# zhuzhui-2000/mobilesuperresolution

Hardware: AMD Instinct MI355X
Metric: HR megapixels/sec (WDSR-B x4, 48x48 LR patches), full training step (higher is better)
Workload: dtype bf16; 1 GPU; WDSR-B x4, 16 blocks / 24 units, 48x48 LR patches, batch 32 per GPU, fwd+L1+bwd+Adam; global_batch=32, parallelism=dp1

## Files before the change

### include/sr_hotpath.h

```cpp
#ifndef SR_HOTPATH_H
#define SR_HOTPATH_H
#include <stddef.h>
#include <stdint.h>

#ifdef __cplusplus
extern "C" {
#endif

typedef void* sr_stream_t;

#define SR_DTYPE_F32 0
#define SR_DTYPE_BF16 1

int sr_abi_version(void);

int sr_wdsr_block_fwd(const void* x, void* y, const void* wblob, const float* cinit,
                      int N, int H, int W, int F, int dtype, sr_stream_t stream);

int sr_wdsr_block2_fwd(const void* x, void* ya, void* yb, const void* wblob_a, const void* wblob_b,
                       const float* cinit_a, const float* cinit_b, void* tsave_a, void* tsave_b, int N, int H, int W,
                       int F, int dtype, sr_stream_t stream);

int sr_wdsr_block2_bwd_data(const void* xa, const void* xb, const void* dyb, void* dxb, void* dxa,
                            const void* wblob_a, const void* wblob_b, const float* cinit_a, const float* cinit_b,
// ... 111 lines not shown

typedef struct { const int* idx; void* out; long src_off, src_stride; int n, reps, as_float; } sr_pack_seg_t;
typedef struct { const float* partial; const int* sidx; const int* dst; long dst_off, dst_stride, slab; int wgs, n, reps; } sr_unpack_seg_t;
int sr_param_pack(const float* flat, float* src, const int* chan_tab, int n_chan, const int* bias_tab, const float* bias_const,
                  int n_bias, const sr_pack_seg_t* segs, int nseg, int dtype, sr_stream_t stream);
int sr_param_grads(const float* flat, float* dsrc, float* gflat, const int* chan_tab, int n_chan, const int* bias_tab,
                   int n_bias, const sr_unpack_seg_t* segs, int nseg, sr_stream_t stream);

typedef struct {
  int F, NB, R, dtype, N, H, W;
  float mean;
  const float* flat; float* gflat;
  const int* chan_tab; int n_chan;
  const int* bias_tab; const float* bias_const; int n_bias;
  float* src; float* dsrc;
  long src_head_off, src_body_off, src_body_stride, src_tail_off;
  const int* idx_head; int n_idx_head;
  const int* idx_body; int n_idx_body;
  const int* idx_cinit; int n_idx_cinit;
  const int* idx_tail; int n_idx_tail;
  void* blob_head; void* blob_body; float* cinit_body; void* blob_tail;
  float* part_a; float* part_b; float* part_tail; float* part_head;
  int wgs_body, wgs_tail, wgs_head;
  int slab_a, slab_b, slab_tail, slab_head;
  const int* ga_sidx; const int* ga_dst; int n_ga;
  const int* gb_sidx; const int* gb_dst; int n_gb;
  const int* gt_sidx; const int* gt_dst; int n_gt;
  const int* gh_sidx; const int* gh_dst; int n_gh;
  const float* x; void* acts; void* grads; float* out; const float* dout;
  void* tsave; void* dtsave;
  const float* hr; int loss_kind; float loss_gscale; float* loss_part;
  int nb_split, chan_split, bias_split;
  int adam_in_wn_bwd;
} sr_wdsr_net_t;

#define SR_NET_SAVE_ACTS 1
#define SR_NET_WEIGHTS_PACKED 2
#define SR_NET_PACK_ONLY 4
int sr_wdsr_net_forward(const sr_wdsr_net_t* net, int flags, sr_stream_t stream);
int sr_wdsr_net_backward(const sr_wdsr_net_t* net, sr_stream_t stream);
int sr_wdsr_net_backward_part(const sr_wdsr_net_t* net, int part, sr_stream_t stream);

int sr_pixel_shuffle(const float* in, float* out, int N, int C, int H, int W, int r, int inverse, sr_stream_t stream);

int sr_tail_bwd_loss(const float* sr, const float* hr, int loss_kind, float gscale, float* loss_part, const void* feat,
                     const float* x_nchw, float mean, const void* wblob, void* dfeat, float* partial, int wgs, int N, int H,
                     int W, int F, int R, int dtype, sr_stream_t stream);

typedef struct { float w_lerp, beta2, one_minus_beta2, bc2_sqrt, eps, neg_step_size; } sr_adam_t;
int sr_adam_step(float* param, const float* grad, float* exp_avg, float* exp_avg_sq, long n, const sr_adam_t* a,
                 const float* loss_part, int n_loss, float loss_scale, float* loss_out, sr_stream_t stream);
int sr_loss_value(const float* loss_part, int n_loss, float loss_scale, float* loss_out, sr_stream_t stream);
int sr_scale_by(void* y, const void* x, long n, const float* scale, int dtype, sr_stream_t stream);
int sr_wdsr_net_train_step(const sr_wdsr_net_t* net, float* exp_avg, float* exp_avg_sq, long n_params, const sr_adam_t* a,
                           float loss_scale, float* loss_out, sr_stream_t stream);

int sr_conv7_fwd(const void* x, const void* wpacked, const float* bias, void* y, int N, int H, int W, int CIN, int COUT, int relu,
                 int out_f32, sr_stream_t stream);

int sr_probe_mfma_bf16(const void* a_frag, const void* b_frag, float* acc_out, sr_stream_t stream);
int sr_probe_mfma_f32(const float* a_frag, const float* b_frag, float* acc_out, sr_stream_t stream);
int sr_probe_tr_read(const void* img_bf16, int n_elems, const int* lane_elem_off, void* out_bf16x4,
                     sr_stream_t stream);
int sr_probe_copy(const void* src, void* dst, size_t n_bytes, sr_stream_t stream);
int sr_probe_launch_floor(void* out, int gx, int gy, int threads, int lds_bytes, int reps, sr_stream_t stream);
int sr_probe_launch_floor_graph(void* out, int gx, int gy, int threads, int lds_bytes, int reps, int iters,
// ... 8 lines not shown
```

### mobilesuperresolution_amd/_lib.py

```python
from __future__ import annotations

import ctypes
import os
from ctypes import c_int, c_size_t, c_void_p

import torch

_HERE = os.path.dirname(os.path.abspath(__file__))
LIB_PATH = os.environ.get("SR_HOTPATH_LIB_PATH") or os.path.join(
    _HERE, "libsr_hotpath_dbg.so" if os.environ.get("SR_HOTPATH_DEBUG_LIB") == "1" else "libsr_hotpath.so")
ABI_VERSION = 13
DTYPE_CODE = {torch.float32: 0, torch.bfloat16: 1}

_P, _I, _Z, _L, _F = c_void_p, c_int, c_size_t, ctypes.c_long, ctypes.c_float
SIGNATURES = {
    "sr_abi_version": ([], _I),
    "sr_wdsr_block_fwd": ([_P, _P, _P, _P, _I, _I, _I, _I, _I, _P], _I),
    "sr_wdsr_block2_fwd": ([_P] * 9 + [_I] * 5 + [_P], _I),
    "sr_wdsr_fwd_rs": ([_P] * 9 + [_I] * 6 + [_P], _I),
    "sr_conv7_fwd": ([_P] * 4 + [_I] * 7 + [_P], _I),
    "sr_wdsr_fwd_rs_repeat": ([_P] * 9 + [_I] * 7 + [_P], _I),
    "sr_wdsr_block_wgrad_saved": ([_P] * 8 + [_I] * 7 + [_L] * 5 + [_P], _I),
    "sr_wdsr_block2_bwd_data": ([_P] * 11 + [_I] * 5 + [_P], _I),
    "sr_wdsr_block2_fwd_repeat": ([_P] * 7 + [_I] * 6 + [_P], _I),
    "sr_probe_launch_floor": ([_P, _I, _I, _I, _I, _I, _P], _I),
    "sr_probe_launch_floor_graph": ([_P, _I, _I, _I, _I, _I, _I, _P, _P], _I),
    "sr_debug_set_stamps": ([_P, _L], _I),
    "sr_c3_trunk_fwd": ([_P] * 6 + [_I] * 7 + [_L, _P], _I),
    "sr_c3_trunk_bwd": ([_P] * 11 + [_I] * 8 + [_L, _P], _I),
    "sr_tail_bwd": ([_P, _P, _P, _F, _P, _P, _P] + [_I] * 7 + [_P], _I),
    "sr_nas_dw_wgrad": ([_P, _P, _P, _P, _I, _I, _I, _I, _I, _I, _P], _I),
    "sr_wdsr_block_fwd_repeat": ([_P, _P, _P, _P, _I, _I, _I, _I, _I, _I, _P], _I),
    "sr_wdsr_block_bwd_data": ([_P, _P, _P, _P, _P, _I, _I, _I, _I, _I, _P], _I),
    "sr_wdsr_block_wgrad": ([_P, _P, _P, _P, _P, _P, _I, _I, _I, _I, _I, _I, _I, _L, _L, _L, _L, _P], _I),
    "sr_wdsr_block_slab_sizes": ([_I, _P, _P], _I),
    "sr_head_fwd": ([_P, _P, _P, _F, _I, _I, _I, _I, _I, _P], _I),
    "sr_tail_fwd": ([_P, _P, _P, _P, _F, _I, _I, _I, _I, _I, _I, _P], _I),
    "sr_tail_bwd_data": ([_P, _P, _P, _I, _I, _I, _I, _I, _I, _P], _I),
    "sr_tail_wgrad": ([_P, _P, _P, _F, _P, _I, _I, _I, _I, _I, _I, _I, _P], _I),
    "sr_head_wgrad": ([_P, _P, _F, _P, _I, _I, _I, _I, _I, _I, _P], _I),
    "sr_c3_fwd": ([_P, _P, _P, _P, _I, _I, _I, _I, _I, _I, _P], _I),
    "sr_c3_bwd_data": ([_P, _P, _P, _P, _P, _I, _I, _I, _I, _I, _I, _P], _I),
    "sr_c3_wgrad": ([_P, _P, _P, _P, _I, _I, _I, _I, _I, _I, _I, _P], _I),
    "sr_flow_warp_fwd": ([_P, _P, _P, _I, _I, _I, _I, _P], _I),
# ... 10 lines not shown
    "sr_nas_body_fwd": ([_P, _P, _P, _L, _P, _L, _P, _L, _P, _L] + [_I] * 6 + [_P], _I),
    "sr_nas_body_bwd": ([_P] * 7 + [_L, _P, _L, _P, _L, _P, _L, _P, _L, _P, _L] + [_I] * 7 + [_P, _P], _I),
    "sr_psnr": ([_P, _P, _P, _P] + [_I] * 7 + [_P], _I),
    "sr_pixel_shuffle": ([_P, _P, _I, _I, _I, _I, _I, _I, _P], _I),
    "sr_tail_bwd_loss": ([_P, _P, _I, _F, _P, _P, _P, _F, _P, _P, _P] + [_I] * 7 + [_P], _I),
    "sr_adam_step": ([_P, _P, _P, _P, _L, _P, _P, _I, _F, _P, _P], _I),
    "sr_loss_value": ([_P, _I, _F, _P, _P], _I),
    "sr_scale_by": ([_P, _P, _L, _P, _I, _P], _I),
    "sr_wdsr_net_train_step": ([_P, _P, _P, _L, _P, _F, _P, _P], _I),
    "sr_wdsr_net_forward": ([_P, _I, _P], _I),
    "sr_wdsr_net_backward": ([_P, _P], _I),
    "sr_wdsr_net_backward_part": ([_P, _I, _P], _I),
    "sr_probe_mfma_bf16": ([_P, _P, _P, _P], _I),
    "sr_probe_mfma_f32": ([_P, _P, _P, _P], _I),
    "sr_probe_tr_read": ([_P, _I, _P, _P, _P], _I),
    "sr_probe_copy": ([_P, _P, _Z, _P], _I),
}

class WdsrNet(ctypes.Structure):
    _fields_ = (
        [(n, _I) for n in ("F", "NB", "R", "dtype", "N", "H", "W")] + [("mean", _F)] +
        [("flat", _P), ("gflat", _P), ("chan_tab", _P), ("n_chan", _I),
         ("bias_tab", _P), ("bias_const", _P), ("n_bias", _I), ("src", _P), ("dsrc", _P)] +
        [(n, _L) for n in ("src_head_off", "src_body_off", "src_body_stride", "src_tail_off")] +
        [("idx_head", _P), ("n_idx_head", _I), ("idx_body", _P), ("n_idx_body", _I),
         ("idx_cinit", _P), ("n_idx_cinit", _I), ("idx_tail", _P), ("n_idx_tail", _I),
         ("blob_head", _P), ("blob_body", _P), ("cinit_body", _P), ("blob_tail", _P),
         ("part_a", _P), ("part_b", _P), ("part_tail", _P), ("part_head", _P)] +
        [(n, _I) for n in ("wgs_body", "wgs_tail", "wgs_head", "slab_a", "slab_b", "slab_tail", "slab_head")] +
        [("ga_sidx", _P), ("ga_dst", _P), ("n_ga", _I), ("gb_sidx", _P), ("gb_dst", _P), ("n_gb", _I),
         ("gt_sidx", _P), ("gt_dst", _P), ("n_gt", _I), ("gh_sidx", _P), ("gh_dst", _P), ("n_gh", _I),
         ("x", _P), ("acts", _P), ("grads", _P), ("out", _P), ("dout", _P), ("tsave", _P), ("dtsave", _P),
         ("hr", _P), ("loss_kind", _I), ("loss_gscale", _F), ("loss_part", _P),
         ("nb_split", _I), ("chan_split", _I), ("bias_split", _I), ("adam_in_wn_bwd", _I)])


class C3Warp(ctypes.Structure):
    _fields_ = [("frame", _P), ("frame_bs", _L), ("state", _P), ("flow", _P), ("flow_bs", _L), ("flow_bound", _P),
                ("dstate", _P), ("dflow", _P), ("dflow_bs", _L), ("x0_save", _P)]


class C3Unpack(ctypes.Structure):
    _fields_ = [("sidx0", _P), ("dst0", _P), ("n0", _I), ("sidx1", _P), ("dst1", _P), ("n1", _I), ("gflat", _P)]


class PackSeg(ctypes.Structure):
    _fields_ = [("idx", _P), ("out", _P), ("src_off", _L), ("src_stride", _L), ("n", _I), ("reps", _I), ("as_float", _I)]


class UnpackSeg(ctypes.Structure):
    _fields_ = [("partial", _P), ("sidx", _P), ("dst", _P), ("dst_off", _L), ("dst_stride", _L), ("slab", _L), ("wgs", _I),
                ("n", _I), ("reps", _I)]


class AdamScalars(ctypes.Structure):
    _fields_ = [(n, _F) for n in ("w_lerp", "beta2", "one_minus_beta2", "bc2_sqrt", "eps", "neg_step_size")]


_lib = None


class HotpathError(RuntimeError):
    pass


def _declare(lib):
    for name, (args, res) in SIGNATURES.items():
# ... 92 lines not shown
```

### mobilesuperresolution_amd/csrc/sr_abi.hip

```cpp
#include <algorithm>
#include <cstdlib>
#include "../../include/sr_hotpath.h"
#include "wdsr_block.h"
#include "wdsr_fwd_rs.h"
#include "wdsr_fwd_stream.h"
#include "wdsr_bwd_rs.h"
#include "wdsr_bwd_pair_lds.h"
#include "wdsr_wgrad_rs.h"
#include "wdsr_ends.h"
#include "wdsr_prep.h"
#include "conv3x3.h"
#include "spynet_conv.h"
#include "nas_block.h"
#include "nas_dw_lc.h"
#include "nas_bwd_fused.h"
#include "flow_warp.h"
#include "metrics.h"
#include "patches.h"
#include "train_step.h"
#include "pixel_shuffle.h"

extern "C" int sr_abi_version(void) { return 13; }

#ifdef SR_DEBUG_STAMPS
#define SR_AB(name) (getenv(name) != nullptr)
#else
#define SR_AB(name) false
#endif

namespace {

template <typename T, int F, int E, int L>
int launch_block_fwd(const void* x, void* y, const void* wblob, const float* cinit, int N, int H, int W,
                     hipStream_t st, void* tsave = nullptr) {
  typedef BlockCfg<F, E, L> C;
  const int tiles_x = (W + C::TW - 1) / C::TW, tiles_y = (H + C::TH - 1) / C::TH;
  dim3 grid(tiles_x * tiles_y, N), block(64 * C::NPT_H);
  hipLaunchKernelGGL((wdsr_block_fwd_kernel<T, F, E, L>), grid, block, 0, st, (const T*)x, (T*)y, (const T*)wblob,
                     cinit, H, W, tiles_x, (T*)tsave);
  SR_HIP_CHECK_LAUNCH();
  return 0;
}

template <typename T, int F, int E, int L>
int launch_block_bwd_data(const void* x, const void* dy, void* dx, const void* wblob, const float* cinit, int N,
                          int H, int W, hipStream_t st, void* dtsave = nullptr) {
  typedef BlockCfg<F, E, L> C;
  const int tiles_x = (W + C::TW - 1) / C::TW, tiles_y = (H + C::TH - 1) / C::TH;
  dim3 grid(tiles_x * tiles_y, N), block(64 * C::NPT_O);
  hipLaunchKernelGGL((wdsr_block_bwd_data_kernel<T, F, E, L>), grid, block, 0, st, (const T*)x, (const T*)dy, (T*)dx,
                     (const T*)wblob, cinit, H, W, tiles_x, (T*)dtsave);
  SR_HIP_CHECK_LAUNCH();
  return 0;
}

// ... 812 lines not shown
                                   n->cinit_body + (size_t)(i + 1) * n->n_idx_cinit, ts ? ts + (size_t)i * side : nullptr,
                                   ts ? ts + (size_t)(i + 1) * side : nullptr, n->N, n->H, n->W, n->F, n->dtype, stream)))
        return rc;
      cur = nxt;
      ++i;
      continue;
    }
    char* nxt = save_acts ? acts + (size_t)(i + 1) * act : (cur == acts ? acts + act : acts);
    if (pairs) {
      char* ts = (save_acts && saved) ? (char*)n->tsave + (size_t)i * side : nullptr;
      if ((rc = sr_wdsr_fwd_rs(cur, nullptr, nxt, (char*)n->blob_body + i * blob, nullptr, n->cinit_body + (size_t)i * n->n_idx_cinit,
                               nullptr, ts, nullptr, 1, n->N, n->H, n->W, n->F, n->dtype, stream)))
        return rc;
      cur = nxt;
      continue;
    }
    if (save_acts && saved) {
      rc = n->F == 24 ? launch_block_fwd<__bf16, 24, 144, 20>(cur, nxt, (char*)n->blob_body + i * blob,
                                                              n->cinit_body + (size_t)i * n->n_idx_cinit, n->N, n->H, n->W,
                                                              st, (char*)n->tsave + (size_t)i * side)
                      : launch_block_fwd<__bf16, 32, 192, 26>(cur, nxt, (char*)n->blob_body + i * blob,
                                                              n->cinit_body + (size_t)i * n->n_idx_cinit, n->N, n->H, n->W,
                                                              st, (char*)n->tsave + (size_t)i * side);
      if (rc) return rc;
    } else if ((rc = sr_wdsr_block_fwd(cur, nxt, (char*)n->blob_body + i * blob,
                                       n->cinit_body + (size_t)i * n->n_idx_cinit, n->N, n->H, n->W, n->F, n->dtype, stream)))
      return rc;
    cur = nxt;
  }
  return sr_tail_fwd(cur, n->x, n->out, n->blob_tail, n->mean, n->N, n->H, n->W, n->F, n->R, n->dtype, stream);
}

namespace {
struct FusedAdam { float* m; float* v; AdamArgs a; const float* loss_part; int n_loss; float loss_scale; float* loss_out; };
}
static int net_backward_part_impl(const sr_wdsr_net_t* n, int part, sr_stream_t stream, const FusedAdam* fa) {
  if (!n || !n->flat || !n->gflat || !n->dsrc || !n->x || !n->acts || !n->grads || part < 0 || part > 2) return -2;
  if (part != 2 && (n->hr ? (!n->out || !n->loss_part || (n->loss_kind != 1 && n->loss_kind != 2)) : !n->dout)) return -2;
  hipStream_t st = (hipStream_t)stream;
  const size_t esz = n->dtype == SR_DTYPE_BF16 ? 2 : 4;
  const size_t act = (size_t)n->N * n->H * n->W * n->F * esz;
  const size_t blob = (size_t)n->n_idx_body * esz;
  const long act_e = (long)n->N * n->H * n->W * n->F;
  char* acts = (char*)n->acts;
  char* grads = (char*)n->grads;
  const bool pairs = net_uses_pairs(n) ||
                     (n->F == 32 && n->dtype == SR_DTYPE_BF16 && net_tiles(n) <= 384 && !getenv("SR_F32_ONE_BLOCK"));
  const bool saved = net_saves_side_images(n, true);
  const size_t side = side_image_bytes(n);
  int split = part == 0 ? 0 : n->nb_split;
  if (part != 0 && (split <= 0 || split >= n->NB || (pairs && ((n->NB - split) & 1)))) return -2;
  const int b0 = part == 1 ? split : 0, b1 = part == 2 ? split : n->NB;
  int rc;
  if (part != 2) {
    if (n->hr) {
      if ((rc = sr_tail_bwd_loss(n->out, n->hr, n->loss_kind, n->loss_gscale, n->loss_part, acts + (size_t)n->NB * act, n->x,
                                 n->mean, n->blob_tail, grads + (size_t)n->NB * act, n->part_tail, n->wgs_tail, n->N, n->H, n->W,
                                 n->F, n->R, n->dtype, stream)))
        return rc;
    } else if (n->dtype == SR_DTYPE_BF16) {
      if ((rc = sr_tail_bwd(n->dout, acts + (size_t)n->NB * act, n->x, n->mean, n->blob_tail, grads + (size_t)n->NB * act,
                            n->part_tail, n->wgs_tail, n->N, n->H, n->W, n->F, n->R, n->dtype, stream)))
        return rc;
    } else {
      if ((rc = sr_tail_bwd_data(n->dout, grads + (size_t)n->NB * act, n->blob_tail, n->N, n->H, n->W, n->F, n->R,
                                 n->dtype, stream)))
        return rc;
// ... 48 lines not shown
        return rc;
    } else if ((rc = sr_wdsr_block_wgrad(a0, g1, wb0, ci0, pa0, pb0, nl, wgs_part, n->N, n->H, n->W, n->F, n->dtype, act_e,
                                         act_e, (long)n->n_idx_body, (long)n->n_idx_cinit, stream)))
      return rc;
  }
  if (part != 1)
    if ((rc = sr_head_wgrad(grads, n->x, n->mean, n->part_head, n->wgs_head, n->N, n->H, n->W, n->F, n->dtype, stream)))
      return rc;
  {
    UnpackSegs us;
    us.nseg = 0;
    int blk = 0;
    auto add = [&](const float* part_, const int* sidx, const int* dst, long off, long stride, long slab, int wgs, int cnt,
                   int reps) {
      us.s[us.nseg++] = UnpackSeg{part_, sidx, dst, off, stride, slab, wgs, cnt, reps, blk};
      blk += reps * unpack_blocks(cnt, wgs);
    };
    if (nl > 0) {
      add(n->part_a, n->ga_sidx, n->ga_dst, n->src_body_off + b0 * n->src_body_stride, n->src_body_stride, n->slab_a, wgs_part,
          n->n_ga, nl);
      add(n->part_b, n->gb_sidx, n->gb_dst, n->src_body_off + b0 * n->src_body_stride, n->src_body_stride, n->slab_b, wgs_part,
          n->n_gb, nl);
    }
    if (part != 2) add(n->part_tail, n->gt_sidx, n->gt_dst, n->src_tail_off, 0, n->slab_tail, n->wgs_tail, n->n_gt, 1);
    if (part != 1) add(n->part_head, n->gh_sidx, n->gh_dst, n->src_head_off, 0, n->slab_head, n->wgs_head, n->n_gh, 1);
    hipLaunchKernelGGL(unpack_all_kernel, dim3(blk), dim3(64 * UNPACK_Q), 0, st, n->dsrc, us);
  }
  const int c0 = part == 1 ? n->chan_split : 0, c1 = part == 2 ? n->chan_split : n->n_chan;
  const int d0 = part == 1 ? n->bias_split : 0, d1 = part == 2 ? n->bias_split : n->n_bias;
  const int cb = (c1 - c0 + 3) / 4, bb = (d1 - d0 + 255) / 256;
  if (fa)
    hipLaunchKernelGGL(wn_bwd_adam_kernel, dim3(cb + bb), dim3(256), 0, st, const_cast<float*>(n->flat), n->dsrc, n->gflat, fa->m, fa->v,
                       (const int4*)n->chan_tab + c0, c1 - c0, n->bias_tab + 3 * d0, d1 - d0, cb, fa->a, fa->loss_part, fa->n_loss,
                       fa->loss_scale, fa->loss_out);
  else
    hipLaunchKernelGGL(wn_bwd_kernel, dim3(cb + bb), dim3(256), 0, st, n->flat, n->dsrc, n->gflat, (const int4*)n->chan_tab + c0,
                       c1 - c0, n->bias_tab + 3 * d0, d1 - d0, cb);
  SR_HIP_CHECK_LAUNCH();
  return 0;
}
extern "C" int sr_wdsr_net_backward_part(const sr_wdsr_net_t* n, int part, sr_stream_t stream) {
  return net_backward_part_impl(n, part, stream, nullptr);
}

extern "C" int sr_wdsr_net_backward(const sr_wdsr_net_t* n, sr_stream_t stream) { return sr_wdsr_net_backward_part(n, 0, stream); }

extern "C" int sr_param_pack(const float* flat, float* src, const int* chan_tab, int n_chan, const int* bias_tab,
                             const float* bias_const, int n_bias, const sr_pack_seg_t* segs, int nseg, int dtype,
                             sr_stream_t stream) {
  if (!flat || !src || !chan_tab || n_chan <= 0 || n_bias < 0 || (n_bias > 0 && (!bias_tab || !bias_const)) || !segs || nseg < 1 ||
      nseg > 4 || (dtype != SR_DTYPE_F32 && dtype != SR_DTYPE_BF16))
    return -2;
  hipStream_t st = (hipStream_t)stream;
  const int cb = (n_chan + 3) / 4, bb = (n_bias + 255) / 256;
  hipLaunchKernelGGL(wn_src_kernel, dim3(cb + bb), dim3(256), 0, st, flat, src, (const int4*)chan_tab, n_chan, bias_tab, bias_const,
                     n_bias, cb);
  PackSegs ps;
  ps.nseg = nseg;
  int blk = 0;
  for (int k = 0; k < nseg; ++k) {
    const sr_pack_seg_t& g = segs[k];
    if (!g.idx || !g.out || g.n <= 0 || g.reps <= 0) return -2;
    ps.s[k] = PackSeg{g.idx, g.out, g.src_off, g.src_stride, g.n, g.reps, g.as_float, blk};
    blk += g.reps * ((g.n + 255) / 256);
  }
  if (dtype == SR_DTYPE_BF16) hipLaunchKernelGGL((pack_all_kernel<__bf16>), dim3(blk), dim3(256), 0, st, src, ps);
  else hipLaunchKernelGGL((pack_all_kernel<float>), dim3(blk), dim3(256), 0, st, src, ps);
// ... 169 lines not shown
}

extern "C" int sr_adam_step(float* p, const float* g, float* m, float* v, long n, const sr_adam_t* a, const float* loss_part,
                            int n_loss, float loss_scale, float* loss_out, sr_stream_t stream) {
  if (!p || !g || !m || !v || !a || n <= 0 || (loss_out && (!loss_part || n_loss <= 0))) return -2;
  const AdamArgs aa{a->w_lerp, a->beta2, a->one_minus_beta2, a->bc2_sqrt, a->eps, a->neg_step_size};
  const long blocks = (n + 1023) / 1024;
  hipLaunchKernelGGL(adam_step_kernel, dim3((unsigned)blocks), dim3(256), 0, (hipStream_t)stream, p, g, m, v, n, aa, loss_part, n_loss,
                     loss_scale, loss_out);
  SR_HIP_CHECK_LAUNCH();
  return 0;
}
extern "C" int sr_loss_value(const float* loss_part, int n_loss, float loss_scale, float* loss_out, sr_stream_t stream) {
  if (!loss_part || !loss_out || n_loss <= 0) return -2;
  hipLaunchKernelGGL(loss_sum_kernel, dim3(1), dim3(64), 0, (hipStream_t)stream, loss_part, n_loss, loss_scale, loss_out);
  SR_HIP_CHECK_LAUNCH();
  return 0;
}
extern "C" int sr_scale_by(void* y, const void* x, long n, const float* scale, int dtype, sr_stream_t stream) {
  if (!y || !x || !scale || n <= 0 || ((uintptr_t)y & 15) || ((uintptr_t)x & 15)) return -2;
  const unsigned blocks = (unsigned)((n + 2047) / 2048);
  if (dtype == SR_DTYPE_BF16)
    hipLaunchKernelGGL(scale_by_kernel<__bf16>, dim3(blocks), dim3(256), 0, (hipStream_t)stream, (__bf16*)y, (const __bf16*)x, n, scale);
  else if (dtype == SR_DTYPE_F32)
    hipLaunchKernelGGL(scale_by_kernel<float>, dim3(blocks), dim3(256), 0, (hipStream_t)stream, (float*)y, (const float*)x, n, scale);
  else return -1;
  SR_HIP_CHECK_LAUNCH();
  return 0;
}
extern "C" int sr_wdsr_net_train_step(const sr_wdsr_net_t* n, float* m, float* v, long n_params, const sr_adam_t* a,
                                      float loss_scale, float* loss_out, sr_stream_t stream) {
  if (!n || !n->hr || !m || !v || !a || n_params <= 0) return -2;
  int rc;
  if ((rc = sr_wdsr_net_forward(n, SR_NET_SAVE_ACTS, stream))) return rc;
  static const bool separate = SR_AB("SR_TRAIN_SEPARATE_ADAM");
  if (!separate && n->adam_in_wn_bwd) {
    const FusedAdam fa{m, v, AdamArgs{a->w_lerp, a->beta2, a->one_minus_beta2, a->bc2_sqrt, a->eps, a->neg_step_size}, n->loss_part,
                       n->wgs_tail, loss_scale, loss_out};
    return net_backward_part_impl(n, 0, stream, &fa);
  }
  if ((rc = sr_wdsr_net_backward(n, stream))) return rc;
  return sr_adam_step(const_cast<float*>(n->flat), n->gflat, m, v, n_params, a, n->loss_part, n->wgs_tail, loss_scale, loss_out, stream);
}

__global__ void probe_mfma_bf16_kernel(const bf16x8* a, const bf16x8* b, float* out) {
  const int l = threadIdx.x;
  f32x16 acc = zero16();
  acc = mma16<__bf16>(a[l], b[l], acc);
#pragma unroll
  for (int i = 0; i < 16; ++i) out[l * 16 + i] = acc[i];
}
__global__ void probe_mfma_f32_kernel(const f32x8* a, const f32x8* b, float* out) {
  const int l = threadIdx.x;
  f32x16 acc = zero16();
  acc = mma16<float>(a[l], b[l], acc);
#pragma unroll
  for (int i = 0; i < 16; ++i) out[l * 16 + i] = acc[i];
}
__global__ void probe_tr_kernel(const __bf16* img, int n, const int* off, bf16x4* out) {
  __shared__ __attribute__((aligned(16))) __bf16 lds[8192];
  for (int i = threadIdx.x; i < n && i < 8192; i += 64) lds[i] = img[i];
  __syncthreads();
  typedef __attribute__((address_space(3))) bf16x4 lds_bf16x4;
  out[threadIdx.x] = __builtin_amdgcn_ds_read_tr16_b64_v4bf16((lds_bf16x4*)(lds + off[threadIdx.x]));
}
__global__ void probe_copy_kernel(const u32x4* __restrict__ src, u32x4* __restrict__ dst, size_t n16) {
  for (size_t i = (size_t)blockIdx.x * blockDim.x + threadIdx.x; i < n16; i += (size_t)gridDim.x * blockDim.x)
    dst[i] = src[i];
}

extern "C" int sr_probe_mfma_bf16(const void* a, const void* b, float* out, sr_stream_t stream) {
  hipLaunchKernelGGL(probe_mfma_bf16_kernel, dim3(1), dim3(64), 0, (hipStream_t)stream, (const bf16x8*)a,
                     (const bf16x8*)b, out);
  SR_HIP_CHECK_LAUNCH();
  return 0;
// ... 119 lines not shown
```

### mobilesuperresolution_amd/csrc/train_step.h

```cpp
#pragma once
#include "sr_common.h"

struct AdamArgs {
  float w_lerp, beta2, one_minus_beta2, bc2_sqrt, eps, neg_step_size;
};
__global__ __launch_bounds__(256) void adam_step_kernel(float* __restrict__ p, const float* __restrict__ g,
                                                        float* __restrict__ m, float* __restrict__ v, long n, AdamArgs a,
                                                        const float* __restrict__ loss_part, int n_loss, float loss_scale,
                                                        float* __restrict__ loss_out) {
  const long i0 = ((long)blockIdx.x * 256 + threadIdx.x) * 4;
  if (i0 + 3 < n) {
    const f32x4 gv = *reinterpret_cast<const f32x4*>(g + i0);
    f32x4 mv = *reinterpret_cast<const f32x4*>(m + i0), vv = *reinterpret_cast<const f32x4*>(v + i0);
    f32x4 pv = *reinterpret_cast<const f32x4*>(p + i0);
#pragma unroll
    for (int j = 0; j < 4; ++j) {
      mv[j] = __builtin_fmaf(a.w_lerp, gv[j] - mv[j], mv[j]);
      const float vb = vv[j] * a.beta2;
      vv[j] = __builtin_fmaf(a.one_minus_beta2, gv[j] * gv[j], vb);
      const float d = __builtin_sqrtf(vv[j]) / a.bc2_sqrt + a.eps;
      pv[j] = __builtin_fmaf(a.neg_step_size, mv[j] / d, pv[j]);
    }
    *reinterpret_cast<f32x4*>(m + i0) = mv;
    *reinterpret_cast<f32x4*>(v + i0) = vv;
    *reinterpret_cast<f32x4*>(p + i0) = pv;
  } else {
    for (long i = i0; i < n; ++i) {
      const float gi = g[i];
      const float mi = __builtin_fmaf(a.w_lerp, gi - m[i], m[i]);
      const float vi = __builtin_fmaf(a.one_minus_beta2, gi * gi, v[i] * a.beta2);
      const float d = __builtin_sqrtf(vi) / a.bc2_sqrt + a.eps;
      m[i] = mi;
      v[i] = vi;
      p[i] = __builtin_fmaf(a.neg_step_size, mi / d, p[i]);
// ... 10 lines not shown

__global__ __launch_bounds__(64) void loss_sum_kernel(const float* __restrict__ loss_part, int n_loss, float loss_scale,
                                                      float* __restrict__ loss_out) {
  float s = 0.f;
  for (int i = threadIdx.x; i < n_loss; i += 64) s += loss_part[i];
#pragma unroll
  for (int o = 32; o > 0; o >>= 1) s += __shfl_xor(s, o);
  if (threadIdx.x == 0) *loss_out = s * loss_scale;
}

template <typename T>
__global__ __launch_bounds__(256) void scale_by_kernel(T* __restrict__ y, const T* __restrict__ x, long n, const float* __restrict__ scale) {
  const float s = *scale;
  const long i0 = ((long)blockIdx.x * 256 + threadIdx.x) * 8;
  if (i0 + 8 <= n) {
    typedef T V __attribute__((ext_vector_type(8)));
    V v = *reinterpret_cast<const V*>(x + i0);
#pragma unroll
    for (int j = 0; j < 8; ++j) v[j] = (T)((float)v[j] * s);
    *reinterpret_cast<V*>(y + i0) = v;
  } else {
    for (long i = i0; i < n; ++i) y[i] = (T)((float)x[i] * s);
  }
}

SR_DEV void adam_elem(float& p, float g, float& m, float& v, const AdamArgs& a) {
  m = __builtin_fmaf(a.w_lerp, g - m, m);
  const float vb = v * a.beta2;
  v = __builtin_fmaf(a.one_minus_beta2, g * g, vb);
  const float d = __builtin_sqrtf(v) / a.bc2_sqrt + a.eps;
  p = __builtin_fmaf(a.neg_step_size, m / d, p);
}

__global__ __launch_bounds__(256) void wn_bwd_adam_kernel(float* __restrict__ flat, const float* __restrict__ dsrc,
                                                          float* __restrict__ gflat, float* __restrict__ em, float* __restrict__ ev,
                                                          const int4* __restrict__ chan_tab, int n_chan,
                                                          const int* __restrict__ bias_tab, int n_bias, int chan_blocks, AdamArgs a,
                                                          const float* __restrict__ loss_part, int n_loss, float loss_scale,
                                                          float* __restrict__ loss_out) {
  const int lane = threadIdx.x & 63, wave = threadIdx.x >> 6;
  if (loss_out && blockIdx.x == gridDim.x - 1 && threadIdx.x >= 192) {
    float s = 0.f;
    for (int i = lane; i < n_loss; i += 64) s += loss_part[i];
#pragma unroll
    for (int o = 32; o > 0; o >>= 1) s += __shfl_xor(s, o);
    if (lane == 0) *loss_out = s * loss_scale;
  }
  if ((int)blockIdx.x < chan_blocks) {
    const int c = blockIdx.x * 4 + wave;
    if (c >= n_chan) return;
    const int4 t = chan_tab[c];
    float* v = flat + t.x;
    const float* dw = dsrc + t.w;
    float ss = 0.f, dot = 0.f;
    for (int k = lane; k < t.z; k += 64) { const float x = v[k]; ss += x * x; dot += x * dw[k]; }
#pragma unroll
    for (int o = 32; o > 0; o >>= 1) { ss += __shfl_xor(ss, o); dot += __shfl_xor(dot, o); }
    const float n = sqrtf(ss), g = flat[t.y];
    const float s1 = g / n, s2 = dot / ss;
    for (int k = lane; k < t.z; k += 64) {
      float gk = s1 * (dw[k] - v[k] * s2);
      asm volatile("" : "+v"(gk));
      gflat[t.x + k] = gk;
      float pk = v[k], mk = em[t.x + k], vk = ev[t.x + k];
      adam_elem(pk, gk, mk, vk, a);
      v[k] = pk; em[t.x + k] = mk; ev[t.x + k] = vk;
    }
    if (lane == 0) {
      float gg = dot / n;
      asm volatile("" : "+v"(gg));
      gflat[t.y] = gg;
      float pg = g, mg = em[t.y], vg = ev[t.y];
      adam_elem(pg, gg, mg, vg, a);
      flat[t.y] = pg; em[t.y] = mg; ev[t.y] = vg;
    }
  } else {
    const int i = (blockIdx.x - chan_blocks) * 256 + threadIdx.x;
    if (i >= n_bias) return;
    const int pa = bias_tab[3 * i], pb = bias_tab[3 * i + 1], d = bias_tab[3 * i + 2];
    const float gval = dsrc[d];
    gflat[pa] = gval;
    { float pp = flat[pa], mm = em[pa], vv = ev[pa]; adam_elem(pp, gval, mm, vv, a); flat[pa] = pp; em[pa] = mm; ev[pa] = vv; }
    if (pb >= 0) {
      gflat[pb] = gval;
      float pp = flat[pb], mm = em[pb], vv = ev[pb];
      adam_elem(pp, gval, mm, vv, a);
      flat[pb] = pp; em[pb] = mm; ev[pb] = vv;
    }
  }
}
```

### mobilesuperresolution_amd/layout.py

```python
from __future__ import annotations

from collections import OrderedDict
from dataclasses import dataclass
from functools import lru_cache

import numpy as np

from . import packing as P


@dataclass(frozen=True)
class ConvSpec:
    name: str
    cout: int
    cin: int
    k: int


class WDSRLayout:
    def __init__(self, F: int, NB: int, R: int):
        self.F, self.NB, self.R = F, NB, R
        E, L = int(F * 6), int(F * 0.84)
        self.E, self.L = E, L
        CO = 3 * R * R
        self.CO = CO
        convs = [ConvSpec("head", F, 3, 3)]
        for i in range(NB):
            convs += [ConvSpec(f"body.{i}.body.0", E, F, 1), ConvSpec(f"body.{i}.body.2", L, E, 1),
                      ConvSpec(f"body.{i}.body.3", F, L, 3)]
        convs += [ConvSpec("tail", CO, F, 3), ConvSpec("skip.0", CO, 3, 5)]
        self.convs = convs
        entries, off = OrderedDict(), 0
        for c in convs:
            for suffix, shape in (("bias", (c.cout,)), ("weight_g", (c.cout, 1, 1, 1)),
                                  ("weight_v", (c.cout, c.cin, c.k, c.k))):
                n = int(np.prod(shape))
                entries[f"{c.name}.{suffix}"] = (off, shape)
# ... 51 lines not shown
            ones.append(base + ob["one"])
            zeros.append(base + ob["zero"])
        self.src_ones, self.src_zeros = np.asarray(ones), np.asarray(zeros)

        bt_ = P.block_tables(F, E, L)
        et_ = P.ends_tables(F, R)
        self.idx_head = et_["head"].astype(np.int32)
        self.idx_tail = et_["tail"].astype(np.int32)
        self.idx_body = bt_["w"].astype(np.int32)
        self.idx_cinit = bt_["cinit"].astype(np.int32)

        gt = P.block_grad_tables(F, E, L)
        n_w1, n_w2, n_w3 = E * F, L * E, F * L * 9
        ga, gb = gt["a"], gt["b"]
        dst_a = np.concatenate([ob["w1"] + np.arange(n_w1), ob["w2"] + np.arange(n_w2),
                                ob["b1"] + np.arange(E), ob["b2"] + np.arange(L)])
        dst_b = np.concatenate([ob["w3"] + np.arange(n_w3), ob["b3"] + np.arange(F)])
        def by_slab(sidx, dst):
            o = np.argsort(sidx, kind="stable")
            return sidx[o].astype(np.int32), dst[o].astype(np.int32)
        self.ga = by_slab(ga, dst_a)
        self.gb = by_slab(gb, dst_b)
        self.slab_a, self.slab_b = gt["a_size"], gt["b_size"]
        ge = P.ends_grad_tables(F, R)
        n_t = CO * F * 9 + CO * 75 + CO
        dst_t = np.concatenate([ot["wt"] + np.arange(CO * F * 9), ot["ws"] + np.arange(CO * 75),
                                ot["b"] + np.arange(CO)])
        assert ge["tail"].size == n_t
        self.gt = by_slab(ge["tail"], dst_t)
        dst_h = np.concatenate([oh["wh"] + np.arange(F * 27), oh["b"] + np.arange(F)])
        self.gh = by_slab(ge["head"], dst_h)
        self.slab_tail, self.slab_head = ge["tail_size"], ge["head_size"]


    def split_at(self, nb_split: int):
        per_block = sum(c.cout for c in self.convs if c.name.startswith("body.0."))
        head_rows = next(c.cout for c in self.convs if c.name == "head")
        first = min(off for name, (off, _) in self.entries.items() if name.startswith(f"body.{nb_split}."))
        return first, head_rows + nb_split * per_block, head_rows + nb_split * per_block


@lru_cache(maxsize=None)
def get_layout(F: int, NB: int, R: int) -> WDSRLayout:
    return WDSRLayout(F, NB, R)
```

### mobilesuperresolution_amd/models/basic_wdsr_b.py

```python
from __future__ import annotations

import ctypes
import math
import os
from collections import OrderedDict

import numpy as np
import torch
import torch.nn as nn

from .. import _lib as L
from ..layout import get_layout

__all__ = ["BASIC_MODEL"]

_DTYPES = {"fp32": torch.float32, "float32": torch.float32, "bf16": torch.bfloat16, "bfloat16": torch.bfloat16}


def _hot_dtype(params) -> torch.dtype:
    name = getattr(params, "hot_dtype", None) or os.environ.get("SR_HOT_DTYPE", "fp32")
    if isinstance(name, torch.dtype):
        return name
    return _DTYPES[str(name).lower()]

# ... 31 lines not shown
        n.F, n.NB, n.R, n.dtype, n.mean = lay.F, lay.NB, lay.R, L.DTYPE_CODE[dt], model.image_mean
        n.chan_tab, n.n_chan = self.chan_tab.data_ptr(), lay.chan_tab.shape[0]
        n.bias_tab, n.bias_const, n.n_bias = self.bias_tab.data_ptr(), self.bias_const.data_ptr(), lay.bias_tab.shape[0]
        n.src, n.dsrc = self.src.data_ptr(), self.dsrc.data_ptr()
        n.src_head_off, n.src_body_off = lay.src_head_off, lay.src_body_off
        n.src_body_stride, n.src_tail_off = lay.src_body_stride, lay.src_tail_off
        for k in ("head", "body", "cinit", "tail"):
            setattr(n, "idx_" + k, self.idx[k].data_ptr())
            setattr(n, "n_idx_" + k, self.idx[k].numel())
        n.blob_head, n.blob_body = self.blob_head.data_ptr(), self.blob_body.data_ptr()
        n.cinit_body, n.blob_tail = self.cinit_body.data_ptr(), self.blob_tail.data_ptr()
        n.part_a, n.part_b = self.part_a.data_ptr(), self.part_b.data_ptr()
        n.part_tail, n.part_head = self.part_tail.data_ptr(), self.part_head.data_ptr()
        n.wgs_body, n.wgs_tail, n.wgs_head = self.wgs_body, self.wgs_tail, self.wgs_head
        n.slab_a, n.slab_b, n.slab_tail, n.slab_head = lay.slab_a, lay.slab_b, lay.slab_tail, lay.slab_head
        for k in ("ga", "gb", "gt", "gh"):
            setattr(n, k + "_sidx", self.g[k][0].data_ptr())
            setattr(n, k + "_dst", self.g[k][1].data_ptr())
            setattr(n, "n_" + k, self.g[k][0].numel())
        n.loss_part = self.loss_part.data_ptr()
        ct, bt = lay.chan_tab, lay.bias_tab
        cover = np.zeros(int(model.flat.numel()), dtype=np.int32)
        for v_off, g_off, K, _dst in ct:
            cover[v_off:v_off + K] += 1
            cover[g_off] += 1
        for a_, b_, _d in bt:
            cover[a_] += 1
            if b_ >= 0:
                cover[b_] += 1
        n.adam_in_wn_bwd = int(bool((cover == 1).all()))
        if model.nb_split:
            _, n.chan_split, n.bias_split = lay.split_at(model.nb_split)
            n.nb_split = model.nb_split
        self.net = n

    def call_struct(self) -> "L.WdsrNet":
        return L.WdsrNet.from_buffer_copy(self.net)


class BASIC_MODEL(nn.Module):

    def __init__(self, params):
        super().__init__()
        self.image_mean = float(params.image_mean)
        self.scale = int(params.scale)
        self.remain_blocks = params.num_blocks
        nin = int(params.num_channels)
        f = int(params.num_residual_units)
        nb = int(params.num_blocks)
        self.num_residual_units, self.num_blocks = f, nb
        if nin != 3 or f not in (24, 32) or self.scale not in (2, 3, 4) or nb < 1:
            raise NotImplementedError(
                "MI355X hot path supports num_channels=3, num_residual_units in {24,32}, scale in {2,3,4} "
                f"(got {nin}, {f}, {self.scale}); there is no generic fallback")
        self.hot_dtype = _hot_dtype(params)
        self.wgs_body = int(getattr(params, "hot_wgs_body", os.environ.get("SR_WGS_BODY", 16)))
        self.layout = get_layout(f, nb, self.scale)
        self.grad_segments = int(getattr(params, "hot_grad_segments", None) or os.environ.get("SR_GRAD_SEGMENTS", 1))
        if self.grad_segments not in (1, 2):
            raise NotImplementedError("hot_grad_segments must be 1 or 2")
        init = self._reference_init()
        self.nb_split = nb - 2 * ((nb // 2 + 1) // 2) if nb >= 2 else 0
        if self.grad_segments == 2 and nb >= 2:
            k = self.layout.split_at(self.nb_split)[0]
            self.flat_lo = nn.Parameter(init[:k])
            self.flat_hi = nn.Parameter(init[k:])
# ... 230 lines not shown
            return 25.0
        return 0.5 * min(self.flat_lo.numel(), self.flat_hi.numel()) * 4 / (1 << 20)

    def make_train_state(self, lr: float = 1e-3, betas=(0.9, 0.999), eps: float = 1e-8):
        return AdamState(self.flat, lr, betas, eps)

    def train_step(self, x: torch.Tensor, hr: torch.Tensor, state: "AdamState", kind: str = "l1", weight: float = 1.0,
                   process_group=None, overlap=None):
        x, hr = self._check_target(x, hr)
        if state.exp_avg.device != x.device:
            raise L.HotpathError("optimizer state and input on different devices")
        st = self._state(x.device)
        flat = self.flat.detach()
        lay = self.layout
        n, _, h, w = x.shape
        if self.grad_segments == 2:
            raise NotImplementedError("train_step is the single-GPU fused step; with hot_grad_segments = 2 train through "
                                      "DistributedDataParallel (forward / loss / backward / optimizer)")
        acts = torch.empty((lay.NB + 1, n, h, w, lay.F), dtype=self.hot_dtype, device=x.device)
        grads = torch.empty_like(acts)
        out = torch.empty((n, 3, self.scale * h, self.scale * w), dtype=torch.float32, device=x.device)
        gflat = torch.empty_like(flat)
        side = dtsave = None
        if self._saves_side_images():
            side = torch.empty(self._side_shape(n, h, w), dtype=self.hot_dtype, device=x.device)
            dtsave = torch.empty_like(side)
        net = st.call_struct()
        net.N, net.H, net.W = n, h, w
        net.flat, net.gflat, net.x = flat.data_ptr(), gflat.data_ptr(), x.data_ptr()
        net.acts, net.grads, net.out = acts.data_ptr(), grads.data_ptr(), out.data_ptr()
        net.tsave = side.data_ptr() if side is not None else None
        net.dtsave = dtsave.data_ptr() if dtsave is not None else None
        net.hr, net.loss_kind, net.loss_gscale = hr.data_ptr(), self._LOSS_KINDS[kind], self._gscale(weight, out.numel())
        loss = torch.empty((), dtype=torch.float32, device=x.device)
        scal = state.next_scalars()
        import torch.distributed as dist
        pg = process_group
        if pg is None and dist.is_available() and dist.is_initialized() and dist.get_world_size() > 1:
            pg = dist.group.WORLD
        with L.device_guard(x.device):
            sp = L.stream_ptr(x.device)
            if overlap is None:
                overlap = flat.numel() >= self.DP_OVERLAP_MIN_PARAMS
            if pg is None:
                L.launch("sr_wdsr_net_train_step", L.lib().sr_wdsr_net_train_step, ctypes.byref(net), state.exp_avg.data_ptr(),
                         state.exp_avg_sq.data_ptr(), flat.numel(), ctypes.byref(scal), float(weight) / out.numel(),
                         loss.data_ptr(), sp)
            elif not (overlap and self.nb_split):
                lib = L.lib()
                L.launch("sr_wdsr_net_forward", lib.sr_wdsr_net_forward, ctypes.byref(net), 1, sp)
                L.launch("sr_wdsr_net_backward_part", lib.sr_wdsr_net_backward_part, ctypes.byref(net), 0, sp)
                avg = dist.get_backend(pg) == "nccl"
                dist.all_reduce(gflat, op=dist.ReduceOp.AVG if avg else dist.ReduceOp.SUM, group=pg)
                if not avg:
                    gflat.div_(dist.get_world_size(pg))
                L.launch("sr_adam_step", lib.sr_adam_step, flat.data_ptr(), gflat.data_ptr(), state.exp_avg.data_ptr(),
                         state.exp_avg_sq.data_ptr(), flat.numel(), ctypes.byref(scal), st.loss_part.data_ptr(), st.wgs_tail,
                         float(weight) / out.numel(), loss.data_ptr(), sp)
            else:
                k = lay.split_at(self.nb_split)[0]
                lib = L.lib()
                L.launch("sr_wdsr_net_forward", lib.sr_wdsr_net_forward, ctypes.byref(net), 1, sp)
                L.launch("sr_wdsr_net_backward_part", lib.sr_wdsr_net_backward_part, ctypes.byref(net), 1, sp)
                avg = dist.get_backend(pg) == "nccl"
                op = dist.ReduceOp.AVG if avg else dist.ReduceOp.SUM
                h_hi = dist.all_reduce(gflat[k:], op=op, group=pg, async_op=True)
                L.launch("sr_wdsr_net_backward_part", lib.sr_wdsr_net_backward_part, ctypes.byref(net), 2, sp)
                if os.environ.get("SR_DP_LAST_ASYNC") == "1":
                    h_lo = dist.all_reduce(gflat[:k], op=op, group=pg, async_op=True)
                    h_hi.wait()
                    h_lo.wait()
                else:
                    h_hi.wait()
                    dist.all_reduce(gflat[:k], op=op, group=pg)
                if not avg:
                    gflat.div_(dist.get_world_size(pg))
                L.launch("sr_adam_step", lib.sr_adam_step, flat.data_ptr(), gflat.data_ptr(), state.exp_avg.data_ptr(),
                         state.exp_avg_sq.data_ptr(), flat.numel(), ctypes.byref(scal), st.loss_part.data_ptr(), st.wgs_tail,
                         float(weight) / out.numel(), loss.data_ptr(), sp)
        _bump_version(self.flat)
        st.packed_key = None
        return loss


def _bump_version(t: torch.Tensor):
    try:
        torch.autograd.graph.increment_version(t)
    except AttributeError:
        t.data.add_(0)


class AdamState:

    def __init__(self, flat: torch.Tensor, lr: float, betas, eps: float):
        self.lr, self.beta1, self.beta2, self.eps = float(lr), float(betas[0]), float(betas[1]), float(eps)
        self.step = 0
        self.exp_avg = torch.zeros_like(flat, memory_format=torch.preserve_format).detach()
        self.exp_avg_sq = torch.zeros_like(self.exp_avg)

    def next_scalars(self) -> "L.AdamScalars":
        self.step += 1
        bc1 = 1.0 - self.beta1 ** self.step
        bc2 = 1.0 - self.beta2 ** self.step
        return L.AdamScalars(1.0 - self.beta1, self.beta2, 1.0 - self.beta2, math.sqrt(bc2), self.eps, -(self.lr / bc1))

    def state_dict(self):
        return {"step": self.step, "exp_avg": self.exp_avg, "exp_avg_sq": self.exp_avg_sq, "lr": self.lr,
                "betas": (self.beta1, self.beta2), "eps": self.eps}

    def load_state_dict(self, d):
        self.step, self.lr, self.eps = int(d["step"]), float(d["lr"]), float(d["eps"])
        self.beta1, self.beta2 = (float(b) for b in d["betas"])
        self.exp_avg.copy_(d["exp_avg"])
        self.exp_avg_sq.copy_(d["exp_avg_sq"])
# ... 122 lines not shown
```

### mobilesuperresolution_amd/packing.py

```python
from __future__ import annotations

from dataclasses import dataclass
from functools import lru_cache
from typing import Dict

import numpy as np

LANES = 64


def _grid(nfrag: int):
    s = np.arange(nfrag).reshape(-1, 1, 1)
    lane = np.arange(LANES).reshape(1, -1, 1)
    j = np.arange(8).reshape(1, 1, -1)
    s, lane, j = np.broadcast_arrays(s, lane, j)
    return s, lane & 31, lane >> 5, j


def k_natural(s, hh, j):
    return 16 * s + 8 * hh + j


def k_chained(s, hh, j):
    return 16 * s + 8 * (j >> 2) + 4 * hh + (j & 3)


def acc_row(i, hh):
    return (i & 3) + 8 * (i >> 2) + 4 * hh


def cinit_index(rows_src: np.ndarray, zero: int) -> np.ndarray:
    hh = np.arange(2).reshape(2, 1)
    i = np.arange(16).reshape(1, 16)
    return rows_src[acc_row(i, hh)].reshape(-1)


@dataclass(frozen=True)
class BlockGeom:
    F: int
    E: int
    L: int

    @property
    def KX(self):
        return self.F if self.F % 16 == 0 else (self.F // 16 + 1) * 16

    @property
    def fold_b1(self):
        return self.F % 16 != 0

    @property
    def KS1(self):
        return self.KX // 16

    @property
    def NET(self):
        return (self.E + 31) // 32

    @property
    def KS2(self):
        return (self.E + 15) // 16

    @property
    def LP(self):
        return ((self.L + 1 + 7) // 8) * 8

    @property
# ... 416 lines not shown
```

Before: 3606 HR-Mpix/s.

## Fold bf16 weight packing into fused weight-norm Adam kernel epilogue

Adds a precomputed scatter table that maps each weight-norm source element to up to four positions in the packed bf16 head/body/tail blobs and the cinit buffer. After the Adam update, the fused wn_bwd_adam kernel recomputes the channel norm, writes the normalized weights, and scatters them straight into the packed blobs. The next forward pass can then skip its separate packing step (weights_packed flag). This removes a pack pass per step, at the cost of extra table loads, a second norm reduction and scattered bf16 stores inside the Adam kernel.

```diff
diff --git a/include/sr_hotpath.h b/include/sr_hotpath.h
--- a/include/sr_hotpath.h
+++ b/include/sr_hotpath.h
@@ -167,6 +167,8 @@
   const float* hr; int loss_kind; float loss_gscale; float* loss_part;
   int nb_split, chan_split, bias_split;
   int adam_in_wn_bwd;
+  const int* pk_tab;
+  int weights_packed;
 } sr_wdsr_net_t;
 
 #define SR_NET_SAVE_ACTS 1
diff --git a/mobilesuperresolution_amd/_lib.py b/mobilesuperresolution_amd/_lib.py
--- a/mobilesuperresolution_amd/_lib.py
+++ b/mobilesuperresolution_amd/_lib.py
@@ -9,7 +9,7 @@
 _HERE = os.path.dirname(os.path.abspath(__file__))
 LIB_PATH = os.environ.get("SR_HOTPATH_LIB_PATH") or os.path.join(
     _HERE, "libsr_hotpath_dbg.so" if os.environ.get("SR_HOTPATH_DEBUG_LIB") == "1" else "libsr_hotpath.so")
-ABI_VERSION = 13
+ABI_VERSION = 14
 DTYPE_CODE = {torch.float32: 0, torch.bfloat16: 1}
 
 _P, _I, _Z, _L, _F = c_void_p, c_int, c_size_t, ctypes.c_long, ctypes.c_float
@@ -86,7 +86,8 @@
          ("gt_sidx", _P), ("gt_dst", _P), ("n_gt", _I), ("gh_sidx", _P), ("gh_dst", _P), ("n_gh", _I),
          ("x", _P), ("acts", _P), ("grads", _P), ("out", _P), ("dout", _P), ("tsave", _P), ("dtsave", _P),
          ("hr", _P), ("loss_kind", _I), ("loss_gscale", _F), ("loss_part", _P),
-         ("nb_split", _I), ("chan_split", _I), ("bias_split", _I), ("adam_in_wn_bwd", _I)])
+         ("nb_split", _I), ("chan_split", _I), ("bias_split", _I), ("adam_in_wn_bwd", _I),
+         ("pk_tab", _P), ("weights_packed", _I)])
 
 
 class C3Warp(ctypes.Structure):
diff --git a/mobilesuperresolution_amd/csrc/sr_abi.hip b/mobilesuperresolution_amd/csrc/sr_abi.hip
--- a/mobilesuperresolution_amd/csrc/sr_abi.hip
+++ b/mobilesuperresolution_amd/csrc/sr_abi.hip
@@ -20,7 +20,7 @@
 #include "train_step.h"
 #include "pixel_shuffle.h"
 
-extern "C" int sr_abi_version(void) { return 13; }
+extern "C" int sr_abi_version(void) { return 14; }
 
 #ifdef SR_DEBUG_STAMPS
 #define SR_AB(name) (getenv(name) != nullptr)
@@ -899,7 +899,7 @@
 }
 
 namespace {
-struct FusedAdam { float* m; float* v; AdamArgs a; const float* loss_part; int n_loss; float loss_scale; float* loss_out; };
+struct FusedAdam { float* m; float* v; AdamArgs a; const float* loss_part; int n_loss; float loss_scale; float* loss_out; PackFold pf; };
 }
 static int net_backward_part_impl(const sr_wdsr_net_t* n, int part, sr_stream_t stream, const FusedAdam* fa) {
   if (!n || !n->flat || !n->gflat || !n->dsrc || !n->x || !n->acts || !n->grads || part < 0 || part > 2) return -2;
@@ -1014,7 +1014,7 @@
   if (fa)
     hipLaunchKernelGGL(wn_bwd_adam_kernel, dim3(cb + bb), dim3(256), 0, st, const_cast<float*>(n->flat), n->dsrc, n->gflat, fa->m, fa->v,
                        (const int4*)n->chan_tab + c0, c1 - c0, n->bias_tab + 3 * d0, d1 - d0, cb, fa->a, fa->loss_part, fa->n_loss,
-                       fa->loss_scale, fa->loss_out);
+                       fa->loss_scale, fa->loss_out, fa->pf);
   else
     hipLaunchKernelGGL(wn_bwd_kernel, dim3(cb + bb), dim3(256), 0, st, n->flat, n->dsrc, n->gflat, (const int4*)n->chan_tab + c0,
                        c1 - c0, n->bias_tab + 3 * d0, d1 - d0, cb);
@@ -1250,15 +1250,25 @@
                                       float loss_scale, float* loss_out, sr_stream_t stream) {
   if (!n || !n->hr || !m || !v || !a || n_params <= 0) return -2;
   int rc;
-  if ((rc = sr_wdsr_net_forward(n, SR_NET_SAVE_ACTS, stream))) return rc;
+  if ((rc = sr_wdsr_net_forward(n, SR_NET_SAVE_ACTS | (n->weights_packed ? SR_NET_WEIGHTS_PACKED : 0), stream))) return rc;
   static const bool separate = SR_AB("SR_TRAIN_SEPARATE_ADAM");
+  const bool fold = n->pk_tab && n->dtype == SR_DTYPE_BF16;
   if (!separate && n->adam_in_wn_bwd) {
+    PackFold pf{};
+    if (fold) {
+      const int c_body = n->n_idx_head, c_cinit = c_body + n->NB * n->n_idx_body, c_tail = c_cinit + n->NB * n->n_idx_cinit;
+      pf = PackFold{(const int4*)n->pk_tab, n->bias_const, n->src, (__bf16*)n->blob_head, (__bf16*)n->blob_body, n->cinit_body,
+                    (__bf16*)n->blob_tail, c_body, c_cinit, c_tail};
+    }
     const FusedAdam fa{m, v, AdamArgs{a->w_lerp, a->beta2, a->one_minus_beta2, a->bc2_sqrt, a->eps, a->neg_step_size}, n->loss_part,
-                       n->wgs_tail, loss_scale, loss_out};
+                       n->wgs_tail, loss_scale, loss_out, pf};
     return net_backward_part_impl(n, 0, stream, &fa);
   }
   if ((rc = sr_wdsr_net_backward(n, stream))) return rc;
-  return sr_adam_step(const_cast<float*>(n->flat), n->gflat, m, v, n_params, a, n->loss_part, n->wgs_tail, loss_scale, loss_out, stream);
+  if ((rc = sr_adam_step(const_cast<float*>(n->flat), n->gflat, m, v, n_params, a, n->loss_part, n->wgs_tail, loss_scale, loss_out,
+                         stream)))
+    return rc;
+  return fold ? net_pack<__bf16>(n, (hipStream_t)stream) : 0;
 }
 
 __global__ void probe_mfma_bf16_kernel(const bf16x8* a, const bf16x8* b, float* out) {
diff --git a/mobilesuperresolution_amd/csrc/train_step.h b/mobilesuperresolution_amd/csrc/train_step.h
--- a/mobilesuperresolution_amd/csrc/train_step.h
+++ b/mobilesuperresolution_amd/csrc/train_step.h
@@ -1,5 +1,6 @@
 #pragma once
 #include "sr_common.h"
+#include "wdsr_prep.h"
 
 struct AdamArgs {
   float w_lerp, beta2, one_minus_beta2, bc2_sqrt, eps, neg_step_size;
@@ -76,12 +77,33 @@
   p = __builtin_fmaf(a.neg_step_size, m / d, p);
 }
 
+struct PackFold {
+  const int4* tab; const float* bias_const; float* src;
+  __bf16* head; __bf16* body; float* cinit; __bf16* tail;
+  int c_body, c_cinit, c_tail;
+};
+constexpr int FOLD_U = 6;
+SR_DEV void fold_put(const PackFold& f, int c, float val) {
+  if (c < 0) return;
+  if (c < f.c_body) f.head[c] = (__bf16)val;
+  else if (c < f.c_cinit) f.body[c - f.c_body] = (__bf16)val;
+  else if (c < f.c_tail) f.cinit[c - f.c_cinit] = val;
+  else f.tail[c - f.c_tail] = (__bf16)val;
+}
+SR_DEV void fold_store(const PackFold& f, int s, float val, int4 row) {
+  f.src[s] = val;
+  fold_put(f, row.x, val);
+  fold_put(f, row.y, val);
+  fold_put(f, row.z, val);
+  fold_put(f, row.w, val);
+}
+
 __global__ __launch_bounds__(256) void wn_bwd_adam_kernel(float* __restrict__ flat, const float* __restrict__ dsrc,
                                                           float* __restrict__ gflat, float* __restrict__ em, float* __restrict__ ev,
                                                           const int4* __restrict__ chan_tab, int n_chan,
                                                           const int* __restrict__ bias_tab, int n_bias, int chan_blocks, AdamArgs a,
                                                           const float* __restrict__ loss_part, int n_loss, float loss_scale,
-                                                          float* __restrict__ loss_out) {
+                                                          float* __restrict__ loss_out, PackFold pf) {
   const int lane = threadIdx.x & 63, wave = threadIdx.x >> 6;
   if (loss_out && blockIdx.x == gridDim.x - 1 && threadIdx.x >= 192) {
     float s = 0.f;
@@ -94,6 +116,11 @@
     const int c = blockIdx.x * 4 + wave;
     if (c >= n_chan) return;
     const int4 t = chan_tab[c];
+    int4 row[FOLD_U];
+    if (pf.tab) {
+#pragma unroll
+      for (int u = 0; u < FOLD_U; ++u) row[u] = pf.tab[t.w + min(lane + 64 * u, t.z - 1)];
+    }
     float* v = flat + t.x;
     const float* dw = dsrc + t.w;
     float ss = 0.f, dot = 0.f;
@@ -110,26 +137,42 @@
       adam_elem(pk, gk, mk, vk, a);
       v[k] = pk; em[t.x + k] = mk; ev[t.x + k] = vk;
     }
+    float gg = dot / n;
+    asm volatile("" : "+v"(gg));
+    float pg = g, mg = em[t.y], vg = ev[t.y];
+    adam_elem(pg, gg, mg, vg, a);
     if (lane == 0) {
-      float gg = dot / n;
-      asm volatile("" : "+v"(gg));
       gflat[t.y] = gg;
-      float pg = g, mg = em[t.y], vg = ev[t.y];
-      adam_elem(pg, gg, mg, vg, a);
       flat[t.y] = pg; em[t.y] = mg; ev[t.y] = vg;
+    }
+    if (pf.tab) {
+      float ss2 = 0.f;
+      for (int k = lane; k < t.z; k += 64) { const float x = v[k]; ss2 += x * x; }
+      ss2 = wave_sum(ss2);
+      const float scale = pg / sqrtf(ss2);
+#pragma unroll
+      for (int u = 0; u < FOLD_U; ++u) {
+        const int k = lane + 64 * u;
+        if (k < t.z) fold_store(pf, t.w + k, v[k] * scale, row[u]);
+      }
+      for (int k = lane + 64 * FOLD_U; k < t.z; k += 64) fold_store(pf, t.w + k, v[k] * scale, pf.tab[t.w + k]);
     }
   } else {
     const int i = (blockIdx.x - chan_blocks) * 256 + threadIdx.x;
     if (i >= n_bias) return;
     const int pa = bias_tab[3 * i], pb = bias_tab[3 * i + 1], d = bias_tab[3 * i + 2];
+    const int4 row = pf.tab ? pf.tab[d] : int4{-1, -1, -1, -1};
     const float gval = dsrc[d];
     gflat[pa] = gval;
-    { float pp = flat[pa], mm = em[pa], vv = ev[pa]; adam_elem(pp, gval, mm, vv, a); flat[pa] = pp; em[pa] = mm; ev[pa] = vv; }
+    float pa_new = flat[pa], pb_new = 0.f;
+    { float mm = em[pa], vv = ev[pa]; adam_elem(pa_new, gval, mm, vv, a); flat[pa] = pa_new; em[pa] = mm; ev[pa] = vv; }
     if (pb >= 0) {
       gflat[pb] = gval;
-      float pp = flat[pb], mm = em[pb], vv = ev[pb];
-      adam_elem(pp, gval, mm, vv, a);
-      flat[pb] = pp; em[pb] = mm; ev[pb] = vv;
+      float mm = em[pb], vv = ev[pb];
+      pb_new = flat[pb];
+      adam_elem(pb_new, gval, mm, vv, a);
+      flat[pb] = pb_new; em[pb] = mm; ev[pb] = vv;
     }
+    if (pf.tab) fold_store(pf, d, pa_new + (pb >= 0 ? pb_new : 0.f) + pf.bias_const[i], row);
   }
 }
diff --git a/mobilesuperresolution_amd/layout.py b/mobilesuperresolution_amd/layout.py
--- a/mobilesuperresolution_amd/layout.py
+++ b/mobilesuperresolution_amd/layout.py
@@ -2,7 +2,7 @@
 
 from collections import OrderedDict
 from dataclasses import dataclass
-from functools import lru_cache
+from functools import cached_property, lru_cache
 
 import numpy as np
 
@@ -120,6 +120,16 @@
         self.gh = by_slab(ge["head"], dst_h)
         self.slab_tail, self.slab_head = ge["tail_size"], ge["head_size"]
 
+    @cached_property
+    def pack_scatter(self):
+        keep = np.zeros(self.src_total, dtype=bool)
+        for _v, _g, K, dst in self.chan_tab:
+            keep[dst:dst + K] = True
+        keep[self.bias_tab[:, 2]] = True
+        return P.scatter_table(self.src_total, [(self.idx_head, self.src_head_off, 0, 1),
+                                                (self.idx_body, self.src_body_off, self.src_body_stride, self.NB),
+                                                (self.idx_cinit, self.src_body_off, self.src_body_stride, self.NB),
+                                                (self.idx_tail, self.src_tail_off, 0, 1)], keep)
 
     def split_at(self, nb_split: int):
         per_block = sum(c.cout for c in self.convs if c.name.startswith("body.0."))
diff --git a/mobilesuperresolution_amd/models/basic_wdsr_b.py b/mobilesuperresolution_amd/models/basic_wdsr_b.py
--- a/mobilesuperresolution_amd/models/basic_wdsr_b.py
+++ b/mobilesuperresolution_amd/models/basic_wdsr_b.py
@@ -87,6 +87,10 @@
         if model.nb_split:
             _, n.chan_split, n.bias_split = lay.split_at(model.nb_split)
             n.nb_split = model.nb_split
+        self.pk = None
+        if dt == torch.bfloat16 and lay.pack_scatter is not None:
+            self.pk = t(lay.pack_scatter)
+            n.pk_tab = self.pk.data_ptr()
         self.net = n
 
     def call_struct(self) -> "L.WdsrNet":
@@ -383,6 +387,7 @@
         net.tsave = side.data_ptr() if side is not None else None
         net.dtsave = dtsave.data_ptr() if dtsave is not None else None
         net.hr, net.loss_kind, net.loss_gscale = hr.data_ptr(), self._LOSS_KINDS[kind], self._gscale(weight, out.numel())
+        net.weights_packed = int(st.pk is not None and st.packed_key == (flat.data_ptr(), flat._version))
         loss = torch.empty((), dtype=torch.float32, device=x.device)
         scal = state.next_scalars()
         import torch.distributed as dist
@@ -430,7 +435,7 @@
                          state.exp_avg_sq.data_ptr(), flat.numel(), ctypes.byref(scal), st.loss_part.data_ptr(), st.wgs_tail,
                          float(weight) / out.numel(), loss.data_ptr(), sp)
         _bump_version(self.flat)
-        st.packed_key = None
+        st.packed_key = (flat.data_ptr(), flat._version) if pg is None and st.pk is not None else None
         return loss
 
 
diff --git a/mobilesuperresolution_amd/packing.py b/mobilesuperresolution_amd/packing.py
--- a/mobilesuperresolution_amd/packing.py
+++ b/mobilesuperresolution_amd/packing.py
@@ -33,6 +33,32 @@
     hh = np.arange(2).reshape(2, 1)
     i = np.arange(16).reshape(1, 16)
     return rows_src[acc_row(i, hh)].reshape(-1)
+
+
+SCATTER_WIDTH = 4
+
+
+def scatter_table(n_src: int, gathers, keep: np.ndarray, width: int = SCATTER_WIDTH):
+    srcs, codes, c0 = [], [], 0
+    for idx, off, stride, reps in gathers:
+        idx = np.asarray(idx, dtype=np.int64)
+        s = (off + stride * np.arange(reps, dtype=np.int64)[:, None] + idx[None, :]).reshape(-1)
+        c = c0 + np.arange(s.size, dtype=np.int64)
+        srcs.append(s[keep[s]])
+        codes.append(c[keep[s]])
+        c0 += s.size
+    assert c0 < 2 ** 31
+    s, c = np.concatenate(srcs), np.concatenate(codes)
+    o = np.argsort(s, kind="stable")
+    s, c = s[o], c[o]
+    start = np.zeros(n_src + 1, dtype=np.int64)
+    np.cumsum(np.bincount(s, minlength=n_src), out=start[1:])
+    slot = np.arange(s.size) - start[s]
+    if s.size and slot.max() >= width:
+        return None
+    tab = np.full((n_src, width), -1, dtype=np.int32)
+    tab[s, slot] = c
+    return tab
 
 
 @dataclass(frozen=True)
```

New measurement: 3646 HR-Mpix/s (median of 6 runs). 1.01x the previous value.
